# henry123-boy/Dynamicfuion_python

Hardware: AMD Instinct MI355X
Metric: GN iters/sec (640x480, 1.5k-node graph) (higher is better)
Workload: dtype f32; 1 GPU; C2: 640x480 depth, 1500-node graph, 77361-vertex/153600-triangle mesh, block-diagonal LM solve, 1 GN iteration per step from a mid-motion node state (half the ground-truth motion); config=C2, nodes=1500, vertices=77361, triangles=153600, anchors=4, hip_graph=True, steps_per_graph=10, step=snapshot, parallelism=single, replicas_per_gpu=1

## Files before the change

### dynamicfuion_python_amd/_native.py

```python
from __future__ import annotations

import ctypes
import os
import subprocess

import torch

_HERE = os.path.dirname(os.path.abspath(__file__))
LIB_PATH = os.environ.get("NNRT_LIB_PATH") or os.path.join(_HERE, "libnnrt_mi355x.so")
CSRC = os.path.join(_HERE, "csrc")

_lib = None

c_int32, c_int64, c_float, c_void_p, c_double_p = ctypes.c_int32, ctypes.c_int64, ctypes.c_float, ctypes.c_void_p, ctypes.POINTER(ctypes.c_double)


class FitterParams(ctypes.Structure):
    _fields_ = [("max_iteration_count", c_int32), ("iteration_mode_count", c_int32), ("iteration_modes", c_int32 * 16),
                ("minimal_update_threshold", c_float), ("use_perspective_correction", c_int32), ("max_depth", c_float),
                ("use_tukey_penalty_for_data_term", c_int32), ("tukey_penalty_cutoff_cm", c_float),
                ("preconditioning_dampening_factor", c_float), ("arap_term_weight", c_float),
                ("use_huber_penalty_for_arap_term", c_int32), ("huber_penalty_constant", c_float), ("use_hip_graph", c_int32),
                ("ndc_convention", c_int32)]

# ... 13 lines not shown
    "nnrt_build_refine_floor": (c_float, []),
    "nnrt_warp_field_create": (c_int32, [c_void_p, c_int32, c_float, c_int32, c_int32, c_int32, c_int32, c_int32, c_int32, c_void_p,
                                         c_int32, ctypes.POINTER(c_void_p)]),
    "nnrt_warp_field_destroy": (None, [c_void_p]),
    "nnrt_warp_field_node_count": (c_int32, [c_void_p]),
    "nnrt_warp_field_edge_count": (c_int32, [c_void_p]),
    "nnrt_warp_field_layer_counts": (c_int32, [c_void_p, c_void_p]),
    "nnrt_warp_field_get_virtual_node_indices": (c_int32, [c_void_p, c_void_p]),
    "nnrt_warp_field_get_edges": (c_int32, [c_void_p, c_void_p, c_void_p]),
    "nnrt_warp_field_get_node_positions": (c_int32, [c_void_p, c_void_p, c_int32]),
    "nnrt_warp_field_get_node_rotations": (c_int32, [c_void_p, c_void_p, c_int32]),
    "nnrt_warp_field_get_node_translations": (c_int32, [c_void_p, c_void_p, c_int32]),
    "nnrt_warp_field_set_node_rotations": (c_int32, [c_void_p, c_void_p, c_int32]),
    "nnrt_warp_field_set_node_translations": (c_int32, [c_void_p, c_void_p, c_int32]),
    "nnrt_warp_field_get_node_coverage_weights": (c_int32, [c_void_p, c_void_p]),
    "nnrt_warp_field_reset_motion": (c_int32, [c_void_p, c_void_p]),
    "nnrt_fitter_default_params": (None, [c_void_p]),
    "nnrt_fitter_create": (c_int32, [c_void_p, c_int32, ctypes.POINTER(c_void_p)]),
    "nnrt_fitter_destroy": (None, [c_void_p]),
    "nnrt_fitter_fit_to_image": (c_int32, [c_void_p, c_void_p, c_void_p, c_void_p, c_int64, c_void_p, c_int64, c_void_p, c_void_p,
                                           c_int32, c_int32, c_void_p, c_void_p, c_float, c_void_p]),
    "nnrt_fitter_prepare": (c_int32, [c_void_p, c_void_p, c_void_p, c_void_p, c_int64, c_void_p, c_int64, c_void_p, c_void_p,
                                      c_int32, c_int32, c_void_p, c_void_p, c_float, c_void_p]),
    "nnrt_fitter_prepare_point_cloud": (c_int32, [c_void_p, c_void_p, c_void_p, c_void_p, c_int64, c_void_p, c_int64, c_void_p, c_void_p,
                                                  c_int32, c_int32, c_void_p, c_void_p, c_void_p]),
    "nnrt_fitter_fit_to_point_cloud": (c_int32, [c_void_p, c_void_p, c_void_p, c_void_p, c_int64, c_void_p, c_int64, c_void_p, c_void_p,
                                                 c_int32, c_int32, c_void_p, c_void_p, c_void_p]),
    "nnrt_fitter_iterate": (c_int32, [c_void_p, c_void_p, c_int32, c_int32, c_void_p]),
    "nnrt_fitter_iterate_from_identity": (c_int32, [c_void_p, c_void_p, c_int32, c_int32, c_void_p]),
    "nnrt_fitter_graph_count": (c_int32, [c_void_p]),
    "nnrt_fitter_corner_info": (c_int32, [c_void_p, c_void_p]),
    "nnrt_fitter_corner_work": (c_int32, [c_void_p, c_void_p]),
    "nnrt_fitter_get_arrowhead_system": (c_int32, [c_void_p, c_void_p, c_void_p, c_void_p, c_int64, c_int64, c_void_p]),
    "nnrt_fitter_get_warped_mesh": (c_int32, [c_void_p, c_void_p, c_void_p, c_int64, c_void_p]),
    "nnrt_release_arrowhead_plans": (None, []),
    "nnrt_fitter_fit_from_snapshot": (c_int32, [c_void_p, c_void_p, c_int32, c_void_p]),
    "nnrt_fitter_restore_motion": (c_int32, [c_void_p, c_void_p, c_void_p]),
    "nnrt_fitter_snapshot_motion": (c_int32, [c_void_p, c_void_p, c_void_p]),
    "nnrt_fitter_iterate_from_snapshot": (c_int32, [c_void_p, c_void_p, c_int32, c_int32, c_void_p]),
    "nnrt_fitter_iterate_timed": (c_int32, [c_void_p, c_void_p, c_int32, c_int32, c_void_p, c_void_p]),
    "nnrt_fitter_time_kernels": (c_int32, [c_void_p, c_void_p, c_int32, c_int32, c_void_p, c_void_p]),
    "nnrt_fitter_refine_info": (c_int32, [c_void_p, c_void_p, c_void_p]),
    "nnrt_fitter_set_refine_ratio": (c_int32, [c_void_p, c_float]),
    "nnrt_fitter_check": (c_int32, [c_void_p, c_void_p]),
    "nnrt_fitter_get_diagnostics": (c_int32, [c_void_p, c_void_p, c_void_p, c_void_p, c_void_p, c_void_p, c_void_p, c_void_p]),
    "nnrt_fitter_get_anchors": (c_int32, [c_void_p, c_void_p, c_void_p, c_void_p]),
# ... 152 lines not shown
```

### dynamicfuion_python_amd/csrc/capi.hip

```cpp
#include <algorithm>
#include <atomic>
#include <cmath>
#include <cstring>
#include <memory>
#include <mutex>
#include <list>
#include <vector>

#include "fitter_kernels.hpp"
#include "warp_field.hpp"
#include "nnrt_dlpack.h"

namespace nnrt {

namespace {
thread_local std::string g_error;
std::atomic<uint64_t> g_next_warp_field_id{1};
}
void set_error(const std::string& message) { g_error = message; }
const std::string& get_error() { return g_error; }

NdcSetup make_ndc_setup(const double* K, int height, int width, bool consistent) {
	const double fx = K[0], fy = K[4], cx = K[2], cy = K[5];
	const double h = height, w = width;
// ... 318 lines not shown
	hipStream_t work = nullptr;
	hipEvent_t ev_in = nullptr, ev_out = nullptr;
	int64_t V = 0, F = 0;
	int H = 0, W = 0, N = 0, K = 0, E = 0;
	bool prepared = false;
	const nnrt_warp_field* wf = nullptr;
	uint64_t wf_id = 0;
	NdcSetup ndc{};
	Camera pix{};
	WarpExtrinsics extr{};
	DeviceBuffer<float> mesh_p, mesh_n;
	DeviceBuffer<int4> faces4;
	DeviceBuffer<int32_t> anchors;
	DeviceBuffer<uint2> anchors16;
	bool use_anchors16 = false;
	DeviceBuffer<float> weights;
	DeviceBuffer<uint32_t> face_nodes;
	DeviceBuffer<float4> wpos, wnrm;
	DeviceBuffer<float2> jrows;
	DeviceBuffer<float4> mesh_p4, mesh_n4;
	DeviceBuffer<float4> ref_points;
	DeviceBuffer<int> tile_flags, tile_order;
	bool use_tile_order = false;
	bool pix_low_occupancy = false;
	DeviceBuffer<float4> records;
	DeviceBuffer<uint64_t> keys;
	DeviceBuffer<float> residuals;
	DeviceBuffer<uint8_t> residual_mask;
	DeviceBuffer<int32_t> pixel_face;
	DeviceBuffer<double> acc;
	DeviceBuffer<float> edge_jr;
	DeviceBuffer<float> updates, gradient, hessian;
	DeviceBuffer<int> error_flag;
	DeviceBuffer<float> wing, edge_residuals, a_diag, a_dinv, a_dinvb, a_rhs, a_x, a_res, a_dx;
	CornerSolver corner;
	DeviceBuffer<int> a_offsets, a_list, a_tgt_off, a_rhs_off, a_rhs_edges, a_inc_off, a_inc_list, a_inc_slot;
	DeviceBuffer<int2> a_tgt_ab, a_pairs;
	ArrowheadWorkspace aw;
	float refine_ratio = NNRT_REFINE_PIVOT_RATIO;
	float refine_ratio_used = NNRT_REFINE_PIVOT_RATIO;
	int n0 = 0;
	int last_mode = 0;
	DeviceBuffer<float> snapshot;
	bool snapshot_valid = false;
	struct SeqGraph {
		std::vector<int> modes;
// ... 81 lines not shown
	fa.pix = ft->pix;
	fa.ndc = ft->ndc;
	fa.blur = ro.blur;
	fa.ax = ro.ax;
	fa.ay = ro.ay;
	fa.perspective = ft->p.use_perspective_correction;
	fa.max_depth = ft->p.max_depth;
	fa.use_tukey = ft->p.use_tukey_penalty_for_data_term;
	fa.tukey_c = ft->p.tukey_penalty_cutoff_cm;
	fa.anchor_count = ft->K;
	fa.keys = ft->keys.ptr;
	fa.faces4 = ft->faces4.ptr;
	fa.wpos = ft->wpos.ptr;
	fa.wnrm = ft->wnrm.ptr;
	fa.anchors = ft->anchors.ptr;
	fa.face_nodes = ft->face_nodes.ptr;
	fa.jrows = ft->jrows.ptr;
	fa.state_in = reinterpret_cast<const float4*>(state_in);
	fa.state_identity = from_identity;
	fa.cmesh_p = ft->mesh_p4.ptr;
	fa.cmesh_n = ft->mesh_n4.ptr;
	fa.weights = ft->weights.ptr;
	fa.ref_points = ft->ref_points.ptr;
	if (ft->use_tile_order) {
		fa.tile_order = ft->tile_order.ptr;
		fa.order_blocks = tile_order_blocks(fa.tiles_x * fa.tiles_y);
	}
	fa.records = ft->records.ptr;
	fa.low_occupancy = ft->pix_low_occupancy ? 1 : 0;
	fa.residuals = ft->residuals.ptr;
	fa.residual_mask = ft->residual_mask.ptr;
	fa.pixel_face = ft->pixel_face.ptr;
	fa.acc = ft->acc.ptr;
	if (ft->E > 0) {
		ArapArgs& aa = fa.arap;
		aa.E = ft->E;
		aa.N = ft->N;
		aa.n0 = ft->n0;
		aa.lambda = ft->p.arap_term_weight;
		aa.use_huber = ft->p.use_huber_penalty_for_arap_term;
		aa.huber_delta = ft->p.huber_penalty_constant;
		aa.coverage_variable = wf->coverage_method == NNRT_MINIMAL_K_NEIGHBOR_NODE_DISTANCE;
		aa.edges = wf->edges.ptr;
		aa.edge_layers = wf->edge_layers.ptr;
		aa.radii = wf->radii.ptr;
		aa.node_weights = wf->node_weights.ptr;
		aa.node_state = state_in;
// ... 72 lines not shown
	auto ft = std::make_unique<nnrt_fitter>();
	ft->p = *params;
	ft->device = device;
	NNRT_HIP(hipStreamCreateWithFlags(&ft->work, hipStreamNonBlocking));
	NNRT_HIP(hipEventCreateWithFlags(&ft->ev_in, hipEventDisableTiming));
	NNRT_HIP(hipEventCreateWithFlags(&ft->ev_out, hipEventDisableTiming));

	nnrt_status st = ft->error_flag.ensure(1);
	if (st) return st;
	NNRT_HIP(hipMemset(ft->error_flag.ptr, 0, sizeof(int)));
	*out = ft.release();
	return NNRT_OK;
}

void nnrt_fitter_destroy(nnrt_fitter* ft) {
	if (!ft) return;
	DeviceGuard guard(ft->device);
	hipStreamSynchronize(ft->work);
	ft->drop_graphs();
	ft->acc.release();
	ft->ref_points.release();
	ft->tile_flags.release();
	ft->tile_order.release();
	ft->records.release();
	for (auto* b : {&ft->mesh_p, &ft->mesh_n, &ft->weights, &ft->residuals, &ft->edge_jr, &ft->updates, &ft->gradient,
	                &ft->hessian, &ft->wing, &ft->edge_residuals, &ft->a_diag, &ft->a_dinv, &ft->a_dinvb, &ft->a_rhs, &ft->a_x, &ft->a_res, &ft->a_dx})
		b->release();
	ft->faces4.release();
	ft->anchors.release();
	ft->anchors16.release();
	ft->face_nodes.release();
	ft->wpos.release();
	ft->wnrm.release();
	ft->jrows.release();
	ft->mesh_p4.release();
	ft->mesh_n4.release();
	ft->keys.release();
	ft->residual_mask.release();
	ft->pixel_face.release();
	ft->error_flag.release();
	ft->a_offsets.release();
	ft->a_list.release();
	ft->a_tgt_off.release();
	ft->a_rhs_off.release();
	ft->a_rhs_edges.release();
	ft->a_tgt_ab.release();
// ... 19 lines not shown
nnrt_status prepare_frame(nnrt_fitter* ft, nnrt_warp_field* wf, const float* d_vertices, const float* d_normals, int64_t V,
                          const int64_t* d_faces, int64_t F, const FrameReference& ref, int32_t H, int32_t W, const double* h_K,
                          const double* h_E, void* stream) {
	NNRT_CHECK_ARG(ft && wf && d_vertices && d_normals && d_faces && (ref.depth || ref.points) && h_K, "null pointer");
	NNRT_CHECK_ARG(V > 0 && F > 0 && H > 0 && W > 0, "empty mesh or image");
	NNRT_CHECK_ARG(V < (int64_t(1) << 31) && F < (int64_t(1) << 31), "mesh too large for int32 indexing");
	NNRT_CHECK_ARG(ref.depth_scale > 0.f, "depth_scale must be positive");
	NNRT_CHECK_ARG(wf->device == ft->device, "the warp field and the fitter live on different devices");
	DeviceGuard guard(ft->device);
	ft->prepared = false;
	hipStream_t us = static_cast<hipStream_t>(stream);
	const int64_t P = static_cast<int64_t>(H) * W;
	const int N = wf->N, K = wf->anchor_count, E = wf->E();
	NNRT_CHECK_ARG(N >= K, "the warp field has fewer nodes than anchors per vertex");
	NNRT_CHECK_ARG(N < FACE_NODE_MAX_NODES, "node count exceeds the face-node table's 20-bit node field");
	if (E > 0) {
		for (int i = 0; i < ft->p.iteration_mode_count; i++)
			if (ft->p.iteration_modes[i] != NNRT_ITERATION_ALL) {
				set_error("the regularized (ARAP) solve supports IterationMode ALL only (reference A15: the ARAP Hessian is 6x6-only)");
				return NNRT_ERROR_UNSUPPORTED;
			}
	}
	const auto before = std::make_tuple(ft->mesh_p.ptr, ft->faces4.ptr, ft->anchors.ptr, ft->keys.ptr, ft->acc.ptr, ft->wing.ptr, ft->corner.generation,
	                                    ft->face_nodes.ptr, ft->wpos.ptr, ft->mesh_p4.ptr, ft->tile_order.ptr, ft->anchors16.ptr);
	nnrt_status st;
	if ((st = ft->mesh_p.ensure(3 * V)) || (st = ft->mesh_n.ensure(3 * V)) || (st = ft->faces4.ensure(F)) ||
	    (st = ft->anchors.ensure(static_cast<size_t>(V) * K)) || (st = ft->weights.ensure(static_cast<size_t>(V) * K)) ||
	    (st = ft->face_nodes.ensure(static_cast<size_t>(F) * face_node_slots(K))) ||
	    (st = ft->wpos.ensure(V)) || (st = ft->wnrm.ensure(V)) ||
	    (st = ft->jrows.ensure(NNRT_GATHER_ROWS ? 3 * static_cast<size_t>(V) * K : 1)) || (st = ft->mesh_p4.ensure(V)) ||
	    (st = ft->mesh_n4.ensure(V)) || (st = ft->anchors16.ensure(K == 4 && N < 65535 ? static_cast<size_t>(V) : 1)) ||
	    (st = ft->ref_points.ensure(P)) || (st = ft->records.ensure(4 * P)) || (st = ft->keys.ensure(P)) ||
	    (st = ft->residuals.ensure(P)) || (st = ft->residual_mask.ensure(P)) || (st = ft->pixel_face.ensure(P)) ||
	    (st = ft->acc.ensure(static_cast<size_t>(N) * ACC_STRIDE)) ||
	    (st = ft->updates.ensure(static_cast<size_t>(N) * 6)) || (st = ft->gradient.ensure(static_cast<size_t>(N) * 6)) ||
	    (st = ft->hessian.ensure(static_cast<size_t>(N) * 36)))
		return st;
	const size_t tiles = static_cast<size_t>(ceil_div(W, 16)) * static_cast<size_t>(ceil_div(H, 16));
	int cus = 0;
	if (hipDeviceGetAttribute(&cus, hipDeviceAttributeMultiprocessorCount, ft->device) != hipSuccess || cus <= 0) cus = 256;
	const bool multi_round = 4 * tiles > static_cast<size_t>(5 * 4 * cus);
	const bool tile_order = fit_pixels_tile_order_supported() && [&] {
		const char* v = std::getenv("NNRT_TILE_ORDER");
		if (v && *v == '0') return false;
		if (v && *v == '2') return true;
		return multi_round;
	}();
	const bool pix_low = [&] {
		const char* v = std::getenv("NNRT_PIX_WPE4");
		if (v) return *v == '1';
		return multi_round;
	}();
	{
		if (tile_order && ((st = ft->tile_flags.ensure(tiles)) || (st = ft->tile_order.ensure(static_cast<size_t>(tile_order_blocks(static_cast<int>(tiles)))))))
			return st;
	}
	ft->E = E;
	ft->n0 = wf->h.layer_counts.empty() ? N : wf->h.layer_counts[0];
	if (E > 0) {
		const int n0 = ft->n0, m = 6 * (N - n0);
		{
			std::vector<float> cpos(3 * static_cast<size_t>(N - n0));
			for (int a = 0; a < N - n0; a++) {
				const int64_t o = wf->h.virtual_indices.empty() ? n0 + a : wf->h.virtual_indices[static_cast<size_t>(n0 + a)];
				for (int c = 0; c < 3; c++) cpos[3 * static_cast<size_t>(a) + c] = wf->nodes_original[3 * static_cast<size_t>(o) + c];
			}
			if ((st = ft->corner.prepare(wf->h.edges.data(), E, n0, N, cpos.data()))) {
				ft->drop_graphs();
				return st;
			}
		}
		if ((st = ft->wing.ensure(static_cast<size_t>(E) * 36)) || (st = ft->edge_residuals.ensure(3 * static_cast<size_t>(E))) ||
		    (st = ft->a_diag.ensure(static_cast<size_t>(N) * 36)) || (st = ft->a_dinv.ensure(static_cast<size_t>(n0) * 36)) ||
		    (st = ft->a_dinvb.ensure(static_cast<size_t>(E) * 36)) ||
		    (st = ft->edge_jr.ensure(2 * static_cast<size_t>(E) * EDGE_TERMS)) ||
		    (st = ft->a_rhs.ensure(6 * static_cast<size_t>(N))) || (st = ft->a_x.ensure(6 * static_cast<size_t>(N))) ||
// ... 39 lines not shown
		ft->aw.tgt_off = ft->a_tgt_off.ptr;
		ft->aw.tgt_ab = ft->a_tgt_ab.ptr;
		ft->aw.pairs = ft->a_pairs.ptr;
		ft->aw.rhs_off = ft->a_rhs_off.ptr;
		ft->aw.rhs_edges = ft->a_rhs_edges.ptr;
		ft->aw.N = N;
		ft->aw.n0 = n0;
		ft->aw.E = E;
		ft->aw.m = m;
		ft->aw.corner = &ft->corner;
		ft->aw.diag = ft->a_diag.ptr;
		ft->aw.dinv = ft->a_dinv.ptr;
		ft->aw.dinv_b = ft->a_dinvb.ptr;
		ft->aw.rhs = ft->a_rhs.ptr;
		ft->aw.x = ft->a_x.ptr;
		ft->aw.refine = NNRT_ARAP_REFINE != 0;
		ft->aw.refine_ratio = ft->refine_ratio;
		ft->aw.res = ft->a_res.ptr;
		ft->aw.dx = ft->a_dx.ptr;
		ft->aw.edge_offsets = ft->a_offsets.ptr;
		ft->aw.edge_list = ft->a_list.ptr;
	}
	const auto after = std::make_tuple(ft->mesh_p.ptr, ft->faces4.ptr, ft->anchors.ptr, ft->keys.ptr, ft->acc.ptr, ft->wing.ptr, ft->corner.generation,
	                                   ft->face_nodes.ptr, ft->wpos.ptr, ft->mesh_p4.ptr, ft->tile_order.ptr, ft->anchors16.ptr);
	const NdcSetup nndc = make_ndc_setup(h_K, H, W, ft->p.ndc_convention == NNRT_NDC_CONSISTENT);
	const Camera npix = pixel_camera(h_K);
	const WarpExtrinsics ne = make_extrinsics(h_E);
	const bool anchors16 = K == 4 && N < 65535 && [] {
		const char* v = std::getenv("NNRT_ANCHORS16");
		return !(v && *v == '0');
	}();
	if (before != after || ft->use_tile_order != tile_order || ft->pix_low_occupancy != pix_low || ft->use_anchors16 != anchors16 || ft->wf != wf || ft->wf_id != wf->id || ft->V != V || ft->F != F || ft->H != H || ft->W != W || ft->N != N ||
	    ft->K != K || std::memcmp(&nndc, &ft->ndc, sizeof(nndc)) != 0 || std::memcmp(&npix, &ft->pix, sizeof(npix)) != 0 ||
	    std::memcmp(&ne, &ft->extr, sizeof(ne)) != 0)
		ft->drop_graphs();
	ft->use_tile_order = tile_order;
	ft->pix_low_occupancy = pix_low;
	ft->use_anchors16 = anchors16;
	ft->V = V;
	ft->F = F;
	ft->H = H;
	ft->W = W;
	ft->N = N;
	ft->K = K;
	ft->wf = wf;
	ft->wf_id = wf->id;
	ft->ndc = nndc;
	ft->pix = npix;
	ft->extr = ne;
	ft->snapshot_valid = false;
	NNRT_HIP(hipEventRecord(ft->ev_in, us));
	NNRT_HIP(hipStreamWaitEvent(ft->work, ft->ev_in, 0));
	hipStream_t s = ft->work;
	NNRT_HIP(hipMemcpyAsync(ft->mesh_p.ptr, d_vertices, sizeof(float) * 3 * V, hipMemcpyDeviceToDevice, s));
	NNRT_HIP(hipMemcpyAsync(ft->mesh_n.ptr, d_normals, sizeof(float) * 3 * V, hipMemcpyDeviceToDevice, s));
	k_faces_to_int4<<<static_cast<unsigned>(ceil_div(F, 256)), 256, 0, s>>>(d_faces, F, V, ft->p.ndc_convention == NNRT_NDC_CONSISTENT,
	                                                                        ft->faces4.ptr, ft->error_flag.ptr);
	NNRT_LAUNCH_CHECK();
	k_to_float4<<<static_cast<unsigned>(ceil_div(V, 256)), 256, 0, s>>>(d_vertices, d_normals, V, ft->mesh_p4.ptr, ft->mesh_n4.ptr);
	NNRT_LAUNCH_CHECK();
	if ((st = launch_compute_anchors(ft->mesh_p.ptr, V, wf->node_positions.ptr, N, K, wf->coverage,
	                                 wf->coverage_method == NNRT_MINIMAL_K_NEIGHBOR_NODE_DISTANCE ? wf->node_weights.ptr : nullptr,
	                                 wf->threshold ? wf->minimum_valid : 0, ft->anchors.ptr, ft->weights.ptr, s)))
		return st;
	if ((st = launch_face_node_table(ft->faces4.ptr, F, ft->anchors.ptr, K, ft->face_nodes.ptr, s))) return st;
	if (ft->use_anchors16 && (st = launch_pack_anchors16(ft->anchors.ptr, V, ft->anchors16.ptr, s))) return st;
	if (ref.depth)
		k_prepare_reference_depth<<<static_cast<unsigned>(ceil_div(P, 256)), 256, 0, s>>>(ref.depth, ref.mask, H, W, ref.depth_scale,
		                                                                                  ft->p.max_depth, ft->pix, ft->ref_points.ptr);
	else
		k_prepare_reference_points<<<static_cast<unsigned>(ceil_div(P, 256)), 256, 0, s>>>(ref.points, ref.mask, P, ft->ref_points.ptr);
	NNRT_LAUNCH_CHECK();
	if (ft->use_tile_order &&
	    (st = launch_tile_order(ft->ref_points.ptr, H, W, static_cast<int>(ceil_div(W, 16)), static_cast<int>(ceil_div(H, 16)), ft->tile_flags.ptr,
	                            ft->tile_order.ptr, s)))
		return st;
	NNRT_HIP(hipMemsetAsync(ft->keys.ptr, 0xff, sizeof(uint64_t) * P, s));
	NNRT_HIP(hipMemsetAsync(ft->acc.ptr, 0, sizeof(double) * N * ACC_STRIDE, s));
	NNRT_HIP(hipEventRecord(ft->ev_out, s));
	NNRT_HIP(hipStreamWaitEvent(us, ft->ev_out, 0));
	ft->prepared = true;
	return NNRT_OK;
}
}

nnrt_status nnrt_fitter_prepare(nnrt_fitter* ft, nnrt_warp_field* wf, const float* d_vertices, const float* d_normals, int64_t V,
                                const int64_t* d_faces, int64_t F, const float* d_depth, const uint8_t* d_mask, int32_t H, int32_t W,
                                const double* h_K, const double* h_E, float depth_scale, void* stream) {
	FrameReference ref;
	ref.depth = d_depth;
	ref.mask = d_mask;
	ref.depth_scale = depth_scale;
	NNRT_CHECK_ARG(d_depth, "null depth image");
	return prepare_frame(ft, wf, d_vertices, d_normals, V, d_faces, F, ref, H, W, h_K, h_E, stream);
}

nnrt_status nnrt_fitter_prepare_point_cloud(nnrt_fitter* ft, nnrt_warp_field* wf, const float* d_vertices, const float* d_normals,
                                            int64_t V, const int64_t* d_faces, int64_t F, const float* d_points, const uint8_t* d_point_mask,
                                            int32_t H, int32_t W, const double* h_K, const double* h_E, void* stream) {
	FrameReference ref;
	ref.points = d_points;
	ref.mask = d_point_mask;
	NNRT_CHECK_ARG(d_points, "null reference point cloud");
	return prepare_frame(ft, wf, d_vertices, d_normals, V, d_faces, F, ref, H, W, h_K, h_E, stream);
}

namespace {
constexpr int MAX_GRAPH_ITERATIONS = 64;
constexpr size_t MAX_CACHED_GRAPHS = 8;
enum { RESET_NONE = 0, RESET_IDENTITY = 1, RESET_SNAPSHOT = 2, RESET_SNAPSHOT_FIRST = 3 };

bool fold_reset(const nnrt_fitter* ft) { return ft->E == 0 && ft->K <= 4; }
bool fold_snapshot(const nnrt_fitter*) { return true; }

nnrt_status check_frame(const nnrt_fitter* ft, const nnrt_warp_field* wf, const char* who) {
	if (!ft->prepared || ft->wf != wf || ft->wf_id != wf->id) {
		set_error(std::string("nnrt_fitter_prepare must be called with this warp field before ") + who);
// ... 1211 lines not shown
```

### dynamicfuion_python_amd/csrc/fitter_kernels.hip

```cpp
#include "fitter_kernels.hpp"



namespace nnrt {

constexpr int PIX_TILE = 16;
#ifndef NNRT_PIX_WAVES
#define NNRT_PIX_WAVES 4
#endif
constexpr int PIX_WAVES = NNRT_PIX_WAVES;
constexpr int PIX_BLOCK = 64 * PIX_WAVES;
static_assert(PIX_WAVES == 1 || PIX_WAVES == 2 || PIX_WAVES == 4, "waves per workgroup");

__device__ inline int pix_quadrant(const FitPixelArgs& a) {
	if (PIX_WAVES == 4 && a.tile_order) {
		const int b = static_cast<int>(blockIdx.x), per_band = a.order_blocks >> 3;
		return a.tile_order[(b & 7) * per_band + (b >> 3)] * 4 + static_cast<int>(threadIdx.x >> 6);
	}
	const int blocks = (4 * a.tiles_x * a.tiles_y + PIX_WAVES - 1) / PIX_WAVES;
	const int per_xcd = (blocks + 7) / 8;
	const int b = static_cast<int>(blockIdx.x);
	return ((b % 8) * per_xcd + b / 8) * PIX_WAVES + static_cast<int>(threadIdx.x >> 6);
}

template <int MODE>
struct ModeTraits;
template <>
struct ModeTraits<NNRT_ITERATION_ALL> {
	static constexpr int S = 6, NH = 21, NACC = 27;
};
template <>
struct ModeTraits<NNRT_ITERATION_TRANSLATION_ONLY> {
	static constexpr int S = 3, NH = 6, NACC = 9;
};
template <>
struct ModeTraits<NNRT_ITERATION_ROTATION_ONLY> {
	static constexpr int S = 3, NH = 6, NACC = 9;
// ... 830 lines not shown
			while (x > 0 && (static_cast<int64_t>(x) * W) / 8 > m) x--;
			order[x * per_band + (m - static_cast<int>((static_cast<int64_t>(x) * W) / 8))] = q;
			m++;
		} else {
			int x = 7;
			while (x > 0 && (static_cast<int64_t>(x) * I) / 8 > n) x--;
			const int wx = static_cast<int>((static_cast<int64_t>(x + 1) * W) / 8 - (static_cast<int64_t>(x) * W) / 8);
			order[x * per_band + wx + (n - static_cast<int>((static_cast<int64_t>(x) * I) / 8))] = q;
			n++;
		}
	}
}

nnrt_status launch_tile_order(const float4* ref_points, int H, int W, int tiles_x, int tiles_y, int* flags, int* order, hipStream_t stream) {
	const int tiles = tiles_x * tiles_y;
	if (tiles == 0) return NNRT_OK;
	k_tile_flags<<<static_cast<unsigned>(tiles), 64, 0, stream>>>(ref_points, H, W, tiles_x, flags);
	NNRT_LAUNCH_CHECK();
	k_tile_order<<<1, ORDER_THREADS, 0, stream>>>(flags, tiles, order);
	NNRT_LAUNCH_CHECK();
	return NNRT_OK;
}

nnrt_status launch_fit_pixels(int mode, const FitPixelArgs& args, hipStream_t stream, hipEvent_t between) {
	if (between) NNRT_EV(hipEventRecord(between, stream));
	const unsigned grid = static_cast<unsigned>((args.tile_order ? args.order_blocks : ((4 * args.tiles_x * args.tiles_y + PIX_WAVES - 1) / PIX_WAVES + 7) / 8 * 8) +
	                                            args.arap_blocks);
	const bool k4 = args.anchor_count <= 4;
	const bool low = args.low_occupancy != 0;
	switch (mode) {
		case NNRT_ITERATION_ALL:
			if (k4 && low) k_fit_pixels_fused<NNRT_ITERATION_ALL, 4, 4><<<grid, PIX_BLOCK, 0, stream>>>(args);
			else if (k4) k_fit_pixels_fused<NNRT_ITERATION_ALL, 4, 5><<<grid, PIX_BLOCK, 0, stream>>>(args);
			else k_fit_pixels_fused<NNRT_ITERATION_ALL, MAX_ANCHORS, 5><<<grid, PIX_BLOCK, 0, stream>>>(args);
			break;
		case NNRT_ITERATION_TRANSLATION_ONLY:
			if (k4 && low) k_fit_pixels_fused<NNRT_ITERATION_TRANSLATION_ONLY, 4, 4><<<grid, PIX_BLOCK, 0, stream>>>(args);
			else if (k4) k_fit_pixels_fused<NNRT_ITERATION_TRANSLATION_ONLY, 4, 5><<<grid, PIX_BLOCK, 0, stream>>>(args);
			else k_fit_pixels_fused<NNRT_ITERATION_TRANSLATION_ONLY, MAX_ANCHORS, 5><<<grid, PIX_BLOCK, 0, stream>>>(args);
			break;
		case NNRT_ITERATION_ROTATION_ONLY:
			if (k4 && low) k_fit_pixels_fused<NNRT_ITERATION_ROTATION_ONLY, 4, 4><<<grid, PIX_BLOCK, 0, stream>>>(args);
			else if (k4) k_fit_pixels_fused<NNRT_ITERATION_ROTATION_ONLY, 4, 5><<<grid, PIX_BLOCK, 0, stream>>>(args);
			else k_fit_pixels_fused<NNRT_ITERATION_ROTATION_ONLY, MAX_ANCHORS, 5><<<grid, PIX_BLOCK, 0, stream>>>(args);
			break;
		default: set_error("unknown iteration mode"); return NNRT_ERROR_ARGUMENT;
	}
	NNRT_LAUNCH_CHECK();
	return NNRT_OK;
// ... 344 lines not shown
```

### dynamicfuion_python_amd/csrc/fitter_kernels.hpp

```cpp
#pragma once

#include <algorithm>
#include <vector>

#include "kernels.hpp"

namespace nnrt {

#ifndef NNRT_SOLVE_LANES
#define NNRT_SOLVE_LANES 1
#endif
#ifndef NNRT_SOLVE_ACC_LDS
#define NNRT_SOLVE_ACC_LDS 1
#endif
constexpr int ACC_STRIDE = 28;

struct ArapArgs {
	int E, N, n0;
	float lambda;
	int use_huber;
	float huber_delta;
	int coverage_variable;
	const int32_t* edges;
	const int8_t* edge_layers;
// ... 120 lines not shown
	uint64_t* keys;
	const int4* faces4;
	const float4* wpos;
	const float4* wnrm;
	const int32_t* anchors;
	const uint32_t* face_nodes;
	const float2* jrows;
	const float4* state_in;
	int state_identity;
	const float4* cmesh_p;
	const float4* cmesh_n;
	const float* weights;
	const float4* ref_points;
	float* residuals;
	uint8_t* residual_mask;
	int32_t* pixel_face;
	double* acc;
	float4* records;
	int low_occupancy;
	ArapArgs arap;
	int arap_blocks;
	const int* tile_order;
	int order_blocks;
};

struct SolveArgs {
	int N;
	float lm;
	double* acc;
	const float* state_in;
	float* node_state;
	float* updates_out;
	float* gradient_out;
	float* hessian_out;
	int* error_flag;
};

constexpr uint32_t FACE_NODE_NONE = 0xFFFFFFFFu;
constexpr int FACE_NODE_SHIFT = 12;
constexpr int FACE_NODE_MAX_NODES = (1 << 20) - 1;
inline int face_node_slots(int K) { return K <= 4 ? 12 : 3 * MAX_ANCHORS; }
nnrt_status launch_face_node_table(int4* faces4, int64_t F, const int32_t* anchors, int K, uint32_t* out, hipStream_t stream);

nnrt_status launch_fit_pixels(int mode, const FitPixelArgs& args, hipStream_t stream, hipEvent_t between = nullptr);
int fit_pixels_arap_blocks(int E);
int tile_order_blocks(int tiles);
bool fit_pixels_tile_order_supported();
nnrt_status launch_tile_order(const float4* ref_points, int H, int W, int tiles_x, int tiles_y, int* flags, int* order, hipStream_t stream);
nnrt_status launch_solve_update(int mode, const SolveArgs& args, hipStream_t stream, bool from_identity = false);


constexpr int CORNER_NB = 64;
inline int corner_ld(int m) { return (m + CORNER_NB - 1) / CORNER_NB * CORNER_NB; }

struct CornerTask {
	int I, J;
	int slot_t, slot_d;
	int src, nd, np;
	int nreal;
};
struct CornerMap {
	int T;
	const int* tile_slot;
	const int* node_row;
	float* tiles;
	float* sdiag;
};
__device__ inline float* corner_entry(const CornerMap& m, int R, int C) {
	const int slot = m.tile_slot[static_cast<int64_t>(R / CORNER_NB) * m.T + C / CORNER_NB];
	return m.tiles + static_cast<int64_t>(slot) * (CORNER_NB * CORNER_NB) + (R % CORNER_NB) * CORNER_NB + (C % CORNER_NB);
}
// ... 188 lines not shown
```

### include/nnrt_mi355x.h

```cpp
#ifndef NNRT_MI355X_H
#define NNRT_MI355X_H

#include <stdint.h>

#ifdef __cplusplus
extern "C" {
#endif

typedef int32_t nnrt_status;
enum {
	NNRT_OK = 0,
	NNRT_ERROR_ARGUMENT = 1,
	NNRT_ERROR_HIP = 2,
	NNRT_ERROR_NOT_POSITIVE_DEFINITE = 3,
	NNRT_ERROR_UNSUPPORTED = 4,
	NNRT_ERROR_CAPACITY = 5,
	NNRT_ERROR_INTERNAL = 6
};

enum { NNRT_ITERATION_ALL = 0, NNRT_ITERATION_TRANSLATION_ONLY = 1, NNRT_ITERATION_ROTATION_ONLY = 2 };
enum { NNRT_FIXED_NODE_COVERAGE = 0, NNRT_MINIMAL_K_NEIGHBOR_NODE_DISTANCE = 1 };

typedef struct nnrt_warp_field nnrt_warp_field;
typedef struct nnrt_fitter nnrt_fitter;
// ... 36 lines not shown
	int32_t use_huber_penalty_for_arap_term;
	float huber_penalty_constant;
	int32_t use_hip_graph;
	int32_t ndc_convention;
} nnrt_fitter_params;
#define NNRT_NDC_REFERENCE 0
#define NNRT_NDC_CONSISTENT 1
#define NNRT_GRAPH_NEVER 0
#define NNRT_GRAPH_AUTO 1
#define NNRT_GRAPH_ALWAYS 2

void nnrt_fitter_default_params(nnrt_fitter_params* params);
nnrt_status nnrt_fitter_create(const nnrt_fitter_params* params, int32_t device, nnrt_fitter** out);
void nnrt_fitter_destroy(nnrt_fitter* fitter);

nnrt_status nnrt_fitter_fit_to_image(nnrt_fitter* fitter, nnrt_warp_field* warp_field, const float* d_vertices, const float* d_normals,
                                     int64_t vertex_count, const int64_t* d_faces, int64_t face_count, const float* d_depth,
                                     const uint8_t* d_mask, int32_t height, int32_t width, const double* h_K, const double* h_E,
                                     float depth_scale, void* stream);
nnrt_status nnrt_fitter_prepare(nnrt_fitter* fitter, nnrt_warp_field* warp_field, const float* d_vertices, const float* d_normals,
                                int64_t vertex_count, const int64_t* d_faces, int64_t face_count, const float* d_depth,
                                const uint8_t* d_mask, int32_t height, int32_t width, const double* h_K, const double* h_E,
                                float depth_scale, void* stream);
nnrt_status nnrt_fitter_prepare_point_cloud(nnrt_fitter* fitter, nnrt_warp_field* warp_field, const float* d_vertices,
                                            const float* d_normals, int64_t vertex_count, const int64_t* d_faces, int64_t face_count,
                                            const float* d_points, const uint8_t* d_point_mask, int32_t height, int32_t width,
                                            const double* h_K, const double* h_E, void* stream);
nnrt_status nnrt_fitter_fit_to_point_cloud(nnrt_fitter* fitter, nnrt_warp_field* warp_field, const float* d_vertices,
                                           const float* d_normals, int64_t vertex_count, const int64_t* d_faces, int64_t face_count,
                                           const float* d_points, const uint8_t* d_point_mask, int32_t height, int32_t width,
                                           const double* h_K, const double* h_E, void* stream);
nnrt_status nnrt_fitter_iterate(nnrt_fitter* fitter, nnrt_warp_field* warp_field, int32_t first_iteration, int32_t count, void* stream);
nnrt_status nnrt_fitter_iterate_from_identity(nnrt_fitter* fitter, nnrt_warp_field* warp_field, int32_t first_iteration, int32_t count,
                                              void* stream);
int32_t nnrt_fitter_graph_count(const nnrt_fitter* fitter);
nnrt_status nnrt_fitter_corner_info(const nnrt_fitter* fitter, int64_t* h_out);
nnrt_status nnrt_fitter_corner_work(const nnrt_fitter* fitter, int64_t* h_out);
nnrt_status nnrt_fitter_get_warped_mesh(nnrt_fitter* fitter, float* h_positions, float* h_normals, int64_t vertex_count, void* stream);
nnrt_status nnrt_fitter_get_arrowhead_system(nnrt_fitter* fitter, float* h_diag, float* h_wing, float* h_rhs, int64_t node_count,
                                             int64_t edge_count, void* stream);
nnrt_status nnrt_fitter_refine_info(nnrt_fitter* fitter, float* h_out, void* stream);
nnrt_status nnrt_fitter_set_refine_ratio(nnrt_fitter* fitter, float ratio);
nnrt_status nnrt_fitter_snapshot_motion(nnrt_fitter* fitter, nnrt_warp_field* warp_field, void* stream);
nnrt_status nnrt_fitter_iterate_from_snapshot(nnrt_fitter* fitter, nnrt_warp_field* warp_field, int32_t first_iteration, int32_t count,
                                              void* stream);
nnrt_status nnrt_fitter_fit_from_snapshot(nnrt_fitter* fitter, nnrt_warp_field* warp_field, int32_t count, void* stream);
// ... 158 lines not shown
```

Measured before the change: 16770 GN iters/s.

## Schedule fit-pixel waves by per-quadrant work order instead of whole tiles

Adds a per-8x8-quadrant scheduling table built once at prepare time. It counts valid reference pixels per quadrant, packs non-empty quadrants densely across eight bands, and spreads empty ones evenly. Overflow quadrants with the fewest valid pixels are pushed to the tail of each band so the first resident wave slots go to heavier quadrants. The fit-pixel kernel then maps each wave to a quadrant through this table rather than tile order, aiming to cut idle waves on masked pixels and balance load across CUs. This becomes the default when a single round of tiles fits on the device, and it adds three small kernels to prepare plus an extra indirection per wave.

```diff
diff --git a/dynamicfuion_python_amd/_native.py b/dynamicfuion_python_amd/_native.py
--- a/dynamicfuion_python_amd/_native.py
+++ b/dynamicfuion_python_amd/_native.py
@@ -59,6 +59,8 @@
                                            c_int32, c_int32, c_void_p, c_void_p, c_float, c_void_p]),
     "nnrt_fitter_prepare": (c_int32, [c_void_p, c_void_p, c_void_p, c_void_p, c_int64, c_void_p, c_int64, c_void_p, c_void_p,
                                       c_int32, c_int32, c_void_p, c_void_p, c_float, c_void_p]),
+    "nnrt_fit_quad_order_blocks": (c_int32, [c_int32]),
+    "nnrt_fit_quad_order_table": (c_int32, [c_void_p, c_int32, c_int32, c_int32, c_void_p, c_void_p]),
     "nnrt_fitter_prepare_point_cloud": (c_int32, [c_void_p, c_void_p, c_void_p, c_void_p, c_int64, c_void_p, c_int64, c_void_p, c_void_p,
                                                   c_int32, c_int32, c_void_p, c_void_p, c_void_p]),
     "nnrt_fitter_fit_to_point_cloud": (c_int32, [c_void_p, c_void_p, c_void_p, c_void_p, c_int64, c_void_p, c_int64, c_void_p, c_void_p,
diff --git a/dynamicfuion_python_amd/csrc/capi.hip b/dynamicfuion_python_amd/csrc/capi.hip
--- a/dynamicfuion_python_amd/csrc/capi.hip
+++ b/dynamicfuion_python_amd/csrc/capi.hip
@@ -364,6 +364,9 @@
 	DeviceBuffer<float4> ref_points;
 	DeviceBuffer<int> tile_flags, tile_order;
 	bool use_tile_order = false;
+	DeviceBuffer<int> quad_scratch, quad_order;
+	bool use_quad_order = false;
+	int quad_slots = 0;
 	bool pix_low_occupancy = false;
 	DeviceBuffer<float4> records;
 	DeviceBuffer<uint64_t> keys;
@@ -491,7 +494,10 @@
 	fa.cmesh_n = ft->mesh_n4.ptr;
 	fa.weights = ft->weights.ptr;
 	fa.ref_points = ft->ref_points.ptr;
-	if (ft->use_tile_order) {
+	if (ft->use_quad_order) {
+		fa.quad_order = ft->quad_order.ptr;
+		fa.order_blocks = quad_order_blocks(4 * fa.tiles_x * fa.tiles_y);
+	} else if (ft->use_tile_order) {
 		fa.tile_order = ft->tile_order.ptr;
 		fa.order_blocks = tile_order_blocks(fa.tiles_x * fa.tiles_y);
 	}
@@ -610,6 +616,8 @@
 	ft->ref_points.release();
 	ft->tile_flags.release();
 	ft->tile_order.release();
+	ft->quad_scratch.release();
+	ft->quad_order.release();
 	ft->records.release();
 	for (auto* b : {&ft->mesh_p, &ft->mesh_n, &ft->weights, &ft->residuals, &ft->edge_jr, &ft->updates, &ft->gradient,
 	                &ft->hessian, &ft->wing, &ft->edge_residuals, &ft->a_diag, &ft->a_dinv, &ft->a_dinvb, &ft->a_rhs, &ft->a_x, &ft->a_res, &ft->a_dx})
@@ -675,7 +683,7 @@
 			}
 	}
 	const auto before = std::make_tuple(ft->mesh_p.ptr, ft->faces4.ptr, ft->anchors.ptr, ft->keys.ptr, ft->acc.ptr, ft->wing.ptr, ft->corner.generation,
-	                                    ft->face_nodes.ptr, ft->wpos.ptr, ft->mesh_p4.ptr, ft->tile_order.ptr, ft->anchors16.ptr);
+	                                    ft->face_nodes.ptr, ft->wpos.ptr, ft->mesh_p4.ptr, ft->tile_order.ptr, ft->quad_order.ptr, ft->anchors16.ptr);
 	nnrt_status st;
 	if ((st = ft->mesh_p.ensure(3 * V)) || (st = ft->mesh_n.ensure(3 * V)) || (st = ft->faces4.ensure(F)) ||
 	    (st = ft->anchors.ensure(static_cast<size_t>(V) * K)) || (st = ft->weights.ensure(static_cast<size_t>(V) * K)) ||
@@ -693,7 +701,7 @@
 	int cus = 0;
 	if (hipDeviceGetAttribute(&cus, hipDeviceAttributeMultiprocessorCount, ft->device) != hipSuccess || cus <= 0) cus = 256;
 	const bool multi_round = 4 * tiles > static_cast<size_t>(5 * 4 * cus);
-	const bool tile_order = fit_pixels_tile_order_supported() && [&] {
+	const bool tile_order_wanted = fit_pixels_tile_order_supported() && [&] {
 		const char* v = std::getenv("NNRT_TILE_ORDER");
 		if (v && *v == '0') return false;
 		if (v && *v == '2') return true;
@@ -704,7 +712,19 @@
 		if (v) return *v == '1';
 		return multi_round;
 	}();
+	const int quad_slots = 4 * 4 * cus;
+	const bool quad_order = fit_pixels_tile_order_supported() && [&] {
+		const char* v = std::getenv("NNRT_QUAD_ORDER");
+		if (v && *v == '0') return false;
+		if (v && *v == '1') return true;
+		const char* t = std::getenv("NNRT_TILE_ORDER");
+		return !multi_round && !(t && *t == '2');
+	}();
+	const bool tile_order = tile_order_wanted && !quad_order;
 	{
+		if (quad_order && ((st = ft->quad_scratch.ensure(quad_order_scratch(static_cast<int>(4 * tiles)))) ||
+		                   (st = ft->quad_order.ensure(4 * static_cast<size_t>(quad_order_blocks(static_cast<int>(4 * tiles)))))))
+			return st;
 		if (tile_order && ((st = ft->tile_flags.ensure(tiles)) || (st = ft->tile_order.ensure(static_cast<size_t>(tile_order_blocks(static_cast<int>(tiles)))))))
 			return st;
 	}
@@ -790,7 +810,7 @@
 		ft->aw.edge_list = ft->a_list.ptr;
 	}
 	const auto after = std::make_tuple(ft->mesh_p.ptr, ft->faces4.ptr, ft->anchors.ptr, ft->keys.ptr, ft->acc.ptr, ft->wing.ptr, ft->corner.generation,
-	                                   ft->face_nodes.ptr, ft->wpos.ptr, ft->mesh_p4.ptr, ft->tile_order.ptr, ft->anchors16.ptr);
+	                                   ft->face_nodes.ptr, ft->wpos.ptr, ft->mesh_p4.ptr, ft->tile_order.ptr, ft->quad_order.ptr, ft->anchors16.ptr);
 	const NdcSetup nndc = make_ndc_setup(h_K, H, W, ft->p.ndc_convention == NNRT_NDC_CONSISTENT);
 	const Camera npix = pixel_camera(h_K);
 	const WarpExtrinsics ne = make_extrinsics(h_E);
@@ -798,11 +818,13 @@
 		const char* v = std::getenv("NNRT_ANCHORS16");
 		return !(v && *v == '0');
 	}();
-	if (before != after || ft->use_tile_order != tile_order || ft->pix_low_occupancy != pix_low || ft->use_anchors16 != anchors16 || ft->wf != wf || ft->wf_id != wf->id || ft->V != V || ft->F != F || ft->H != H || ft->W != W || ft->N != N ||
+	if (before != after || ft->use_tile_order != tile_order || ft->use_quad_order != quad_order || ft->quad_slots != quad_slots || ft->pix_low_occupancy != pix_low || ft->use_anchors16 != anchors16 || ft->wf != wf || ft->wf_id != wf->id || ft->V != V || ft->F != F || ft->H != H || ft->W != W || ft->N != N ||
 	    ft->K != K || std::memcmp(&nndc, &ft->ndc, sizeof(nndc)) != 0 || std::memcmp(&npix, &ft->pix, sizeof(npix)) != 0 ||
 	    std::memcmp(&ne, &ft->extr, sizeof(ne)) != 0)
 		ft->drop_graphs();
 	ft->use_tile_order = tile_order;
+	ft->use_quad_order = quad_order;
+	ft->quad_slots = quad_slots;
 	ft->pix_low_occupancy = pix_low;
 	ft->use_anchors16 = anchors16;
 	ft->V = V;
@@ -843,6 +865,10 @@
 	    (st = launch_tile_order(ft->ref_points.ptr, H, W, static_cast<int>(ceil_div(W, 16)), static_cast<int>(ceil_div(H, 16)), ft->tile_flags.ptr,
 	                            ft->tile_order.ptr, s)))
 		return st;
+	if (ft->use_quad_order &&
+	    (st = launch_quad_order(ft->ref_points.ptr, H, W, static_cast<int>(ceil_div(W, 16)), static_cast<int>(ceil_div(H, 16)), ft->quad_slots,
+	                            ft->quad_scratch.ptr, ft->quad_order.ptr, s)))
+		return st;
 	NNRT_HIP(hipMemsetAsync(ft->keys.ptr, 0xff, sizeof(uint64_t) * P, s));
 	NNRT_HIP(hipMemsetAsync(ft->acc.ptr, 0, sizeof(double) * N * ACC_STRIDE, s));
 	NNRT_HIP(hipEventRecord(ft->ev_out, s));
@@ -861,6 +887,32 @@
 	ref.depth_scale = depth_scale;
 	NNRT_CHECK_ARG(d_depth, "null depth image");
 	return prepare_frame(ft, wf, d_vertices, d_normals, V, d_faces, F, ref, H, W, h_K, h_E, stream);
+}
+
+int32_t nnrt_fit_quad_order_blocks(int32_t quadrants) { return quadrants > 0 ? quad_order_blocks(quadrants) : 0; }
+
+nnrt_status nnrt_fit_quad_order_table(const uint8_t* h_valid, int32_t H, int32_t W, int32_t slots, int32_t* h_counts, int32_t* h_table) {
+	NNRT_CHECK_ARG(h_valid && h_counts && h_table, "null pointer");
+	NNRT_CHECK_ARG(H > 0 && W > 0 && slots >= 0, "empty image or negative slot count");
+	const int tiles_x = static_cast<int>(ceil_div(W, 16)), tiles_y = static_cast<int>(ceil_div(H, 16)), quadrants = 4 * tiles_x * tiles_y;
+	const size_t P = static_cast<size_t>(H) * W, entries = 4 * static_cast<size_t>(quad_order_blocks(quadrants));
+	std::vector<float4> ref(P);
+	for (size_t p = 0; p < P; p++) ref[p] = make_float4(0.f, 0.f, 1.f, h_valid[p] ? 1.f : 0.f);
+	DeviceBuffer<float4> d_ref;
+	DeviceBuffer<int> d_scratch, d_order;
+	nnrt_status st = NNRT_OK;
+	if (!(st = upload(d_ref, ref)) && !(st = d_scratch.ensure(quad_order_scratch(quadrants))) && !(st = d_order.ensure(entries)) &&
+	    !(st = launch_quad_order(d_ref.ptr, H, W, tiles_x, tiles_y, slots, d_scratch.ptr, d_order.ptr, nullptr))) {
+		if (hipMemcpy(h_counts, d_scratch.ptr, sizeof(int) * quadrants, hipMemcpyDeviceToHost) != hipSuccess ||
+		    hipMemcpy(h_table, d_order.ptr, sizeof(int) * entries, hipMemcpyDeviceToHost) != hipSuccess) {
+			set_error("hipMemcpy failed");
+			st = NNRT_ERROR_HIP;
+		}
+	}
+	d_ref.release();
+	d_scratch.release();
+	d_order.release();
+	return st;
 }
 
 nnrt_status nnrt_fitter_prepare_point_cloud(nnrt_fitter* ft, nnrt_warp_field* wf, const float* d_vertices, const float* d_normals,
diff --git a/dynamicfuion_python_amd/csrc/fitter_kernels.hip b/dynamicfuion_python_amd/csrc/fitter_kernels.hip
--- a/dynamicfuion_python_amd/csrc/fitter_kernels.hip
+++ b/dynamicfuion_python_amd/csrc/fitter_kernels.hip
@@ -13,6 +13,11 @@
 static_assert(PIX_WAVES == 1 || PIX_WAVES == 2 || PIX_WAVES == 4, "waves per workgroup");
 
 __device__ inline int pix_quadrant(const FitPixelArgs& a) {
+	if (PIX_WAVES == 4 && a.quad_order) {
+		const int b = static_cast<int>(blockIdx.x), per_band = a.order_blocks >> 3;
+		const int wave = __builtin_amdgcn_readfirstlane(static_cast<int>(threadIdx.x >> 6));
+		return a.quad_order[((b & 7) * per_band + (b >> 3)) * 4 + wave];
+	}
 	if (PIX_WAVES == 4 && a.tile_order) {
 		const int b = static_cast<int>(blockIdx.x), per_band = a.order_blocks >> 3;
 		return a.tile_order[(b & 7) * per_band + (b >> 3)] * 4 + static_cast<int>(threadIdx.x >> 6);
@@ -889,9 +894,123 @@
 	return NNRT_OK;
 }
 
+__host__ __device__ inline int quad_blocks_per_band(int quadrants) { return ((quadrants + 7) / 8 + 1 + 3) / 4; }
+int quad_order_blocks(int quadrants) { return 8 * quad_blocks_per_band(quadrants); }
+
+__global__ __launch_bounds__(256) void k_quad_flags(const float4* __restrict__ ref, int H, int W, int tiles_x, int* __restrict__ counts) {
+	const int tile = static_cast<int>(blockIdx.x), quad = static_cast<int>(threadIdx.x >> 6), lane = static_cast<int>(threadIdx.x & 63);
+	const int u = (tile % tiles_x) * PIX_TILE + (quad & 1) * 8 + (lane & 7), v = (tile / tiles_x) * PIX_TILE + (quad >> 1) * 8 + (lane >> 3);
+	const bool valid = u < W && v < H && ref[static_cast<int64_t>(v) * W + u].w != 0.f;
+	const unsigned long long b = __ballot(valid);
+	if (lane == 0) counts[tile * 4 + quad] = __popcll(b);
+}
+
+__global__ __launch_bounds__(ORDER_THREADS) void k_quad_order(const int* __restrict__ counts, int quadrants, int* __restrict__ work, int* __restrict__ totals,
+                                                              int* __restrict__ order) {
+	__shared__ int s_w[ORDER_THREADS], s_i[ORDER_THREADS];
+	const int t = static_cast<int>(threadIdx.x);
+	const int per_band = 4 * quad_blocks_per_band(quadrants);
+	for (int i = t; i < 8 * per_band; i += ORDER_THREADS) order[i] = quadrants;
+	const int c = (quadrants + ORDER_THREADS - 1) / ORDER_THREADS, t0 = t * c < quadrants ? t * c : quadrants, t1 = t0 + c < quadrants ? t0 + c : quadrants;
+	int nw = 0, ni = 0;
+	for (int q = t0; q < t1; q++) (counts[q] ? nw : ni)++;
+	s_w[t] = nw;
+	s_i[t] = ni;
+	__syncthreads();
+	for (int d = 1; d < ORDER_THREADS; d <<= 1) {
+		const int aw = t >= d ? s_w[t - d] : 0, ai = t >= d ? s_i[t - d] : 0;
+		__syncthreads();
+		s_w[t] += aw;
+		s_i[t] += ai;
+		__syncthreads();
+	}
+	const int W = s_w[ORDER_THREADS - 1], I = s_i[ORDER_THREADS - 1];
+	int m = s_w[t] - nw, n = s_i[t] - ni;
+	if (t == 0) totals[0] = W;
+	for (int q = t0; q < t1; q++) {
+		if (counts[q]) {
+			work[m++] = q;
+		} else {
+			int x = 7;
+			while (x > 0 && (static_cast<int64_t>(x) * I) / 8 > n) x--;
+			const int wx = static_cast<int>((static_cast<int64_t>(x + 1) * W) / 8 - (static_cast<int64_t>(x) * W) / 8);
+			order[x * per_band + wx + (n - static_cast<int>((static_cast<int64_t>(x) * I) / 8))] = q;
+			n++;
+		}
+	}
+}
+
+__global__ __launch_bounds__(64) void k_quad_place(const int* __restrict__ counts, int quadrants, const int* __restrict__ work, const int* __restrict__ totals,
+                                                   int slots, int* __restrict__ order) {
+	__shared__ int s_hist[65], s_cum[65], s_run[65];
+	const int x = static_cast<int>(blockIdx.x), lane = static_cast<int>(threadIdx.x);
+	const int per_band = 4 * quad_blocks_per_band(quadrants);
+	const int W = totals[0];
+	const int first = static_cast<int>((static_cast<int64_t>(x) * W) / 8), run = static_cast<int>((static_cast<int64_t>(x + 1) * W) / 8) - first;
+	const int share = slots / 8 > 0 ? slots / 8 : 0;
+	const int ov = run > share ? run - share : 0;
+	int* band = order + x * per_band;
+	if (ov == 0) {
+		for (int j = lane; j < run; j += 64) band[j] = work[first + j];
+		return;
+	}
+	for (int i = lane; i < 65; i += 64) {
+		s_hist[i] = 0;
+		s_run[i] = 0;
+	}
+	__syncthreads();
+	for (int j = lane; j < run; j += 64) atomicAdd(&s_hist[counts[work[first + j]]], 1);
+	__syncthreads();
+	if (lane == 0) {
+		int sum = 0;
+		for (int i = 0; i < 65; i++) {
+			s_cum[i] = sum;
+			sum += s_hist[i];
+		}
+	}
+	__syncthreads();
+	int cs = 1;
+	for (int i = 1; i < 65; i++)
+		if (s_cum[i] <= ov) cs = i;
+	const int r = ov - s_cum[cs];
+	int kept = 0;
+	for (int j0 = 0; j0 < run; j0 += 64) {
+		const int j = j0 + lane;
+		const bool on = j < run;
+		const int q = on ? work[first + j] : 0;
+		const int cnt = on ? counts[q] : 0;
+		unsigned long long same = 0ull;
+		for (int i = 0; i < 64; i++)
+			if (__shfl(cnt, i) == cnt) same |= 1ull << i;
+		const unsigned long long below = (1ull << lane) - 1ull;
+		const int k = s_run[cnt] + __popcll(same & below);
+		const bool over = on && (cnt < cs || (cnt == cs && k < r));
+		const unsigned long long stay = __ballot(on && !over);
+		if (over) band[(run - ov) + s_cum[cnt] + k] = q;
+		else if (on) band[kept + __popcll(stay & below)] = q;
+		kept += __popcll(stay);
+		__syncthreads();
+		if (on && (same >> lane) <= 1ull) s_run[cnt] += __popcll(same);
+		__syncthreads();
+	}
+}
+
+nnrt_status launch_quad_order(const float4* ref_points, int H, int W, int tiles_x, int tiles_y, int slots, int* scratch, int* order, hipStream_t stream) {
+	const int tiles = tiles_x * tiles_y, quadrants = 4 * tiles;
+	if (tiles == 0) return NNRT_OK;
+	int *counts = scratch, *work = scratch + quadrants, *totals = scratch + 2 * quadrants;
+	k_quad_flags<<<static_cast<unsigned>(tiles), 256, 0, stream>>>(ref_points, H, W, tiles_x, counts);
+	NNRT_LAUNCH_CHECK();
+	k_quad_order<<<1, ORDER_THREADS, 0, stream>>>(counts, quadrants, work, totals, order);
+	NNRT_LAUNCH_CHECK();
+	k_quad_place<<<8, 64, 0, stream>>>(counts, quadrants, work, totals, slots, order);
+	NNRT_LAUNCH_CHECK();
+	return NNRT_OK;
+}
+
 nnrt_status launch_fit_pixels(int mode, const FitPixelArgs& args, hipStream_t stream, hipEvent_t between) {
 	if (between) NNRT_EV(hipEventRecord(between, stream));
-	const unsigned grid = static_cast<unsigned>((args.tile_order ? args.order_blocks : ((4 * args.tiles_x * args.tiles_y + PIX_WAVES - 1) / PIX_WAVES + 7) / 8 * 8) +
+	const unsigned grid = static_cast<unsigned>((args.tile_order || args.quad_order ? args.order_blocks : ((4 * args.tiles_x * args.tiles_y + PIX_WAVES - 1) / PIX_WAVES + 7) / 8 * 8) +
 	                                            args.arap_blocks);
 	const bool k4 = args.anchor_count <= 4;
 	const bool low = args.low_occupancy != 0;
diff --git a/dynamicfuion_python_amd/csrc/fitter_kernels.hpp b/dynamicfuion_python_amd/csrc/fitter_kernels.hpp
--- a/dynamicfuion_python_amd/csrc/fitter_kernels.hpp
+++ b/dynamicfuion_python_amd/csrc/fitter_kernels.hpp
@@ -166,6 +166,7 @@
 	int arap_blocks;
 	const int* tile_order;
 	int order_blocks;
+	const int* quad_order;
 };
 
 struct SolveArgs {
@@ -191,6 +192,9 @@
 int tile_order_blocks(int tiles);
 bool fit_pixels_tile_order_supported();
 nnrt_status launch_tile_order(const float4* ref_points, int H, int W, int tiles_x, int tiles_y, int* flags, int* order, hipStream_t stream);
+int quad_order_blocks(int quadrants);
+inline size_t quad_order_scratch(int quadrants) { return 2 * static_cast<size_t>(quadrants) + 1; }
+nnrt_status launch_quad_order(const float4* ref_points, int H, int W, int tiles_x, int tiles_y, int slots, int* scratch, int* order, hipStream_t stream);
 nnrt_status launch_solve_update(int mode, const SolveArgs& args, hipStream_t stream, bool from_identity = false);
 
 
diff --git a/include/nnrt_mi355x.h b/include/nnrt_mi355x.h
--- a/include/nnrt_mi355x.h
+++ b/include/nnrt_mi355x.h
@@ -82,6 +82,9 @@
                                 int64_t vertex_count, const int64_t* d_faces, int64_t face_count, const float* d_depth,
                                 const uint8_t* d_mask, int32_t height, int32_t width, const double* h_K, const double* h_E,
                                 float depth_scale, void* stream);
+int32_t nnrt_fit_quad_order_blocks(int32_t quadrants);
+nnrt_status nnrt_fit_quad_order_table(const uint8_t* h_valid, int32_t height, int32_t width, int32_t slots, int32_t* h_counts,
+                                      int32_t* h_table);
 nnrt_status nnrt_fitter_prepare_point_cloud(nnrt_fitter* fitter, nnrt_warp_field* warp_field, const float* d_vertices,
                                             const float* d_normals, int64_t vertex_count, const int64_t* d_faces, int64_t face_count,
                                             const float* d_points, const uint8_t* d_point_mask, int32_t height, int32_t width,
```

After: 17720 GN iters/s (median of 6 runs). 5.7% higher.
